# aszepieniec/stark-anatomy

Measured on AMD Instinct MI355X. Metric: ntt_field_elements_per_sec, higher is better.
Workload: dtype u128; 1 GPU; ntt_fwd_inv_2^20_1gpu; log2n=20, parallelism=single, passes_per_transform=2

## Files before the change

stark-anatomy_amd/csrc/field_asm.cuh:

```cuda
#pragma once

#if defined(__HIP_DEVICE_COMPILE__)
namespace sc {

typedef uint64_t smask_t;

#ifndef SC_HAZ_NOP
#define SC_HAZ_NOP "s_nop 1\n\t"
#endif

__device__ __forceinline__ uint64_t a_mad(uint32_t a, uint32_t b, uint64_t c) {
    uint64_t d; smask_t cy;
    asm("v_mad_u64_u32 %0, %1, %2, %3, %4" : "=v"(d), "=s"(cy) : "v"(a), "v"(b), "v"(c));
    return d;
}
__device__ __forceinline__ uint64_t a_madc(uint32_t a, uint32_t b, uint64_t c, smask_t& cy) {
    uint64_t d;
    asm("v_mad_u64_u32 %0, %1, %2, %3, %4" : "=v"(d), "=s"(cy) : "v"(a), "v"(b), "v"(c));
    return d;
}
__device__ __forceinline__ uint32_t a_add_co(uint32_t x, uint32_t y, smask_t& co) {
    uint32_t s;
    asm("v_add_co_u32_e64 %0, %1, %2, %3" : "=v"(s), "=s"(co) : "v"(x), "v"(y));
    return s;
}
__device__ __forceinline__ uint32_t a_addc(uint32_t x, uint32_t y, smask_t ci, smask_t& co) {
    uint32_t s;
    asm(SC_HAZ_NOP "v_addc_co_u32_e64 %0, %1, %2, %3, %4" : "=v"(s), "=s"(co) : "v"(x), "v"(y), "s"(ci));
    return s;
}
__device__ __forceinline__ uint32_t a_addc_last(uint32_t x, uint32_t y, smask_t ci) {
    uint32_t s; smask_t co;
    asm(SC_HAZ_NOP "v_addc_co_u32_e64 %0, %1, %2, %3, %4" : "=v"(s), "=s"(co) : "v"(x), "v"(y), "s"(ci));
    return s;
}
__device__ __forceinline__ uint32_t a_inc(uint32_t x, smask_t ci) {
    uint32_t s; smask_t co;
    asm(SC_HAZ_NOP "v_addc_co_u32_e64 %0, %1, 0, %2, %3" : "=v"(s), "=s"(co) : "v"(x), "s"(ci));
    return s;
}
__device__ __forceinline__ uint32_t a_sub_co(uint32_t x, uint32_t y, smask_t& bo) {
    uint32_t s;
    asm("v_sub_co_u32_e64 %0, %1, %2, %3" : "=v"(s), "=s"(bo) : "v"(x), "v"(y));
    return s;
}
__device__ __forceinline__ uint32_t a_subb(uint32_t x, uint32_t y, smask_t bi, smask_t& bo) {
    uint32_t s;
    asm(SC_HAZ_NOP "v_subb_co_u32_e64 %0, %1, %2, %3, %4" : "=v"(s), "=s"(bo) : "v"(x), "v"(y), "s"(bi));
    return s;
}
__device__ __forceinline__ uint32_t a_negb(uint32_t y, smask_t bi, smask_t& bo) {
    uint32_t s;
    asm(SC_HAZ_NOP "v_subb_co_u32_e64 %0, %1, 0, %2, %3" : "=v"(s), "=s"(bo) : "v"(y), "s"(bi));
    return s;
}
__device__ __forceinline__ uint32_t a_cnd(uint32_t a, uint32_t b, smask_t sel) {
    uint32_t r;
    asm(SC_HAZ_NOP "v_cndmask_b32_e64 %0, %1, %2, %3" : "=v"(r) : "v"(a), "v"(b), "s"(sel));
    return r;
}

__device__ __forceinline__ void rare_or(smask_t& rare, smask_t c) { asm volatile("s_or_b64 %0, %0, %1" : "+s"(rare) : "s"(c) : "scc"); }
__device__ __forceinline__ bool rare_any_asm(smask_t rare) {
    uint32_t any;
    asm("s_cmp_lg_u64 %1, 0\n\ts_cselect_b32 %0, 1, 0" : "=s"(any) : "s"(rare) : "scc");
    return __builtin_amdgcn_readfirstlane(any) != 0;
}

__device__ __forceinline__ uint32_t lo32(uint64_t x) { return (uint32_t)x; }
__device__ __forceinline__ uint32_t hi32(uint64_t x) { return (uint32_t)(x >> 32); }

static constexpr uint32_t PH3 = 0xCB800000u;

__device__ __forceinline__ Fe a_cond_sub_p(uint32_t r0, uint32_t r1, uint32_t r2, uint32_t r3, smask_t cf) {
    smask_t b;
    uint32_t d0 = a_sub_co(r0, 1u, b);
    uint32_t d1 = a_subb(r1, 0u, b, b);
    uint32_t d2 = a_subb(r2, 0u, b, b);
    uint32_t d3 = a_subb(r3, PH3, b, b);
    smask_t sel = cf | ~b;
    uint32_t o0 = a_cnd(r0, d0, sel), o1 = a_cnd(r1, d1, sel), o2 = a_cnd(r2, d2, sel), o3 = a_cnd(r3, d3, sel);
    return Fe{((uint64_t)o1 << 32) | o0, ((uint64_t)o3 << 32) | o2};
}

__device__ __forceinline__ Fe a_fixup_fast(uint32_t d0, uint32_t d1, uint32_t d2, uint32_t d3, smask_t bw, smask_t& rare) {
    smask_t c;
    const uint32_t d3p = d3 + PH3;
    uint32_t o0 = a_addc(d0, 0u, bw, c);
    uint32_t o3 = a_cnd(d3, d3p, bw);
    rare_or(rare, c);
    return Fe{((uint64_t)d1 << 32) | o0, ((uint64_t)o3 << 32) | d2};
}

#define SC_FIX_CARRY(o1, o2, o3, c)                                                \
    SC_HAZ_NOP "v_addc_co_u32_e64 %[" o1 "], %[t], %[" o1 "], 0, %[" c "]\n\t"      \
    SC_HAZ_NOP "v_addc_co_u32_e64 %[" o2 "], %[t], %[" o2 "], 0, %[t]\n\t"          \
    SC_HAZ_NOP "v_addc_co_u32_e64 %[" o3 "], %[t], %[" o3 "], 0, %[t]\n\t"
#define SC_FIX_BORROW(o0, o1, o2, o3, r3, b, ca)                                   \
    SC_HAZ_NOP "v_subb_co_u32_e64 %[" o1 "], %[t], %[" o1 "], 0, %[" b "]\n\t"      \
    SC_HAZ_NOP "v_subb_co_u32_e64 %[" o2 "], %[t], %[" o2 "], 0, %[t]\n\t"          \
    SC_HAZ_NOP "v_subb_co_u32_e64 %[" o3 "], %[t], %[" o3 "], 0, %[t]\n\t"          \
    "s_andn2_b64 %[t], %[t], %[" ca "]\n\t"                                        \
    SC_HAZ_NOP "v_cndmask_b32_e64 %[" o0 "], %[" o0 "], 0, %[t]\n\t"               \
    "v_cndmask_b32_e64 %[" o1 "], %[" o1 "], 0, %[t]\n\t"                          \
    "v_cndmask_b32_e64 %[" o2 "], %[" o2 "], 0, %[t]\n\t"                          \
    "v_cndmask_b32_e64 %[" o3 "], %[" o3 "], %[" r3 "], %[t]\n\t"

__device__ __forceinline__ Fe a_fixup_fix(uint32_t d0, uint32_t d1, uint32_t d2, uint32_t d3, smask_t bw) {
    smask_t c, t;
    const uint32_t d3p = d3 + PH3;
    uint32_t o0 = a_addc(d0, 0u, bw, c);
    uint32_t o3 = a_cnd(d3, d3p, bw);
    asm("s_cmp_eq_u64 %[c], 0\n\t"
        "s_cbranch_scc1 1f\n\t"
        SC_FIX_CARRY("o1", "o2", "o3", "c")
        "1:"
        : [o1] "+v"(d1), [o2] "+v"(d2), [o3] "+v"(o3), [t] "=&s"(t)
        : [c] "s"(c)
        : "scc");
    return Fe{((uint64_t)d1 << 32) | o0, ((uint64_t)o3 << 32) | d2};
}

template <int MODE>
__device__ __forceinline__ Fe mont_mul_core(Fe a, Fe b, smask_t& rare) {
    const uint32_t a0 = lo32(a.lo), a1 = hi32(a.lo), a2 = lo32(a.hi), a3 = hi32(a.hi);
    const uint32_t b0 = lo32(b.lo), b1 = hi32(b.lo), b2 = lo32(b.hi), b3 = hi32(b.hi);
    smask_t c;
    uint64_t E0 = a_mad(a0, b0, 0);
    uint64_t O0 = a_mad(a0, b1, 0);
    O0 = a_madc(a1, b0, O0, c);
    uint32_t nO0 = a_inc(0u, c);
    uint64_t E1 = a_mad(a0, b2, 0);
    E1 = a_madc(a1, b1, E1, c);
    uint32_t nE1 = a_inc(0u, c);
    E1 = a_madc(a2, b0, E1, c);
    nE1 = a_inc(nE1, c);
    uint64_t O1 = a_mad(a0, b3, (uint64_t)nO0);
    O1 = a_madc(a1, b2, O1, c);
    uint32_t nO1 = a_inc(0u, c);
    O1 = a_madc(a2, b1, O1, c);
    nO1 = a_inc(nO1, c);
    O1 = a_madc(a3, b0, O1, c);
    nO1 = a_inc(nO1, c);
    uint64_t E2 = a_mad(a1, b3, (uint64_t)nE1);
    E2 = a_madc(a2, b2, E2, c);
    uint32_t nE2 = a_inc(0u, c);
    E2 = a_madc(a3, b1, E2, c);
    nE2 = a_inc(nE2, c);
    uint64_t O2 = a_mad(a2, b3, (uint64_t)nO1);
    O2 = a_madc(a3, b2, O2, c);
    uint32_t nO2 = a_inc(0u, c);
    uint64_t E3 = a_mad(a3, b3, (uint64_t)nE2);
    const uint32_t t0 = lo32(E0);
    uint32_t t1 = a_add_co(hi32(E0), lo32(O0), c);
    uint32_t t2 = a_addc(lo32(E1), hi32(O0), c, c);
    uint32_t t3 = a_addc(hi32(E1), lo32(O1), c, c);
    uint32_t t4 = a_addc(lo32(E2), hi32(O1), c, c);
    uint32_t t5 = a_addc(hi32(E2), lo32(O2), c, c);
    uint32_t t6 = a_addc(lo32(E3), hi32(O2), c, c);
    uint32_t t7 = a_addc_last(hi32(E3), nO2, c);
    const uint32_t PHc = PH3;
    uint64_t s0 = a_mad(t0, PHc, 0);
    smask_t bw;
    uint32_t m3 = a_sub_co(t3, lo32(s0), bw);
    uint64_t s1 = a_mad(t1, PHc, (uint64_t)hi32(s0));
    uint64_t s2 = a_mad(t2, PHc, (uint64_t)hi32(s1));
    uint64_t s3 = a_mad(m3, PHc, (uint64_t)hi32(s2));
    uint32_t r0 = a_subb(t4, lo32(s1), bw, bw);
    uint32_t r1 = a_subb(t5, lo32(s2), bw, bw);
    uint32_t r2 = a_subb(t6, lo32(s3), bw, bw);
    uint32_t r3 = a_subb(t7, hi32(s3), bw, bw);
    if constexpr (MODE == 1) return a_fixup_fast(r0, r1, r2, r3, bw, rare);
    if constexpr (MODE == 2) return a_fixup_fix(r0, r1, r2, r3, bw);
    uint32_t ph = a_cnd(0u, PH3, bw);
    uint32_t o0 = a_addc(r0, 0u, bw, c);
    uint32_t o1 = a_addc(r1, 0u, c, c);
    uint32_t o2 = a_addc(r2, 0u, c, c);
    uint32_t o3 = a_addc_last(r3, ph, c);
    return Fe{((uint64_t)o1 << 32) | o0, ((uint64_t)o3 << 32) | o2};
}
__device__ __forceinline__ Fe mont_mul_asm(Fe a, Fe b) {
    smask_t none = 0;
    return mont_mul_core<0>(a, b, none);
}
__device__ __forceinline__ Fe mont_mul_fast_asm(Fe a, Fe b, smask_t& rare) { return mont_mul_core<1>(a, b, rare); }
__device__ __forceinline__ Fe mont_mul_fix_asm(Fe a, Fe b) {
    smask_t none = 0;
    return mont_mul_core<2>(a, b, none);
}

#define SC_V_MAD(d, cy, x, y, c)   asm volatile("v_mad_u64_u32 %0, %1, %2, %3, %4" : "=v"(d), "=s"(cy) : "v"(x), "v"(y), "v"(c))
#define SC_V_INC(d, x, ci, co)     asm volatile("v_addc_co_u32_e64 %0, %1, 0, %2, %3" : "=v"(d), "=s"(co) : "v"(x), "s"(ci))
#define SC_V_ADDCO(d, co, x, y)    asm volatile("v_add_co_u32_e64 %0, %1, %2, %3" : "=v"(d), "=s"(co) : "v"(x), "v"(y))
#define SC_V_ADDC(d, co, x, y, ci) asm volatile("v_addc_co_u32_e64 %0, %1, %2, %3, %4" : "=v"(d), "=s"(co) : "v"(x), "v"(y), "s"(ci))
#define SC_V_SUBCO(d, bo, x, y)    asm volatile("v_sub_co_u32_e64 %0, %1, %2, %3" : "=v"(d), "=s"(bo) : "v"(x), "v"(y))
#define SC_V_SUBB(d, bo, x, y, bi) asm volatile("v_subb_co_u32_e64 %0, %1, %2, %3, %4" : "=v"(d), "=s"(bo) : "v"(x), "v"(y), "s"(bi))
#define SC_V_CND(d, x, y, m)       asm volatile("v_cndmask_b32_e64 %0, %1, %2, %3" : "=v"(d) : "v"(x), "v"(y), "s"(m))
#define SC_V_NOP0()                asm volatile("s_nop 0")

template <int W> __device__ __forceinline__ void v_mad_dump(uint64_t& d, uint32_t x, uint32_t y, uint64_t c) {
    if constexpr (W == 0) asm volatile("v_mad_u64_u32 %0, vcc, %1, %2, %3" : "=v"(d) : "v"(x), "v"(y), "v"(c) : "vcc");
    else asm volatile("v_mad_u64_u32 %0, s[100:101], %1, %2, %3" : "=v"(d) : "v"(x), "v"(y), "v"(c) : "s100", "s101");
}
template <int W> __device__ __forceinline__ void v_inc_dump(uint32_t& d, uint32_t x, smask_t ci) {
    if constexpr (W == 0) asm volatile("v_addc_co_u32_e64 %0, vcc, %1, 0, %2" : "=v"(d) : "v"(x), "s"(ci) : "vcc");
    else asm volatile("v_addc_co_u32_e64 %0, s[100:101], %1, 0, %2" : "=v"(d) : "v"(x), "s"(ci) : "s100", "s101");
}
template <int W> __device__ __forceinline__ void v_addc_dump(uint32_t& d, uint32_t x, uint32_t y, smask_t ci) {
    if constexpr (W == 0) asm volatile("v_addc_co_u32_e64 %0, vcc, %1, %2, %3" : "=v"(d) : "v"(x), "v"(y), "s"(ci) : "vcc");
    else asm volatile("v_addc_co_u32_e64 %0, s[100:101], %1, %2, %3" : "=v"(d) : "v"(x), "v"(y), "s"(ci) : "s100", "s101");
}
#define SC_V_MADD(d, x, y, c)      v_mad_dump<W>(d, x, y, c)
#define SC_V_INCD(d, x, ci)        v_inc_dump<W>(d, x, ci)
#define SC_V_ADDCD(d, x, y, ci)    v_addc_dump<W>(d, x, y, ci)

struct MulState {
    uint32_t a0, a1, a2, a3, b0, b1, b2, b3;
    uint64_t E0, O0, E1, O1, E2, O2, E3, s0, s1, s2, s3;
    uint32_t nO0, nE1, nO1, nE2, nO2, t1, t2, t3, t4, t5, t6, t7, m3, r0, r1, r2, r3, ph, o0, o1, o2, o3;
    smask_t c1, c2, c3, c4, c5, c6, c7, c8, c9, ct, bw, cx;
};

template <int MODE>
__device__ __forceinline__ void mont_mul2_core(Fe xa, Fe wa, Fe xb, Fe wb, Fe& ra, Fe& rb, smask_t& rare) {
    MulState A, B;
    A.a0 = lo32(xa.lo); A.a1 = hi32(xa.lo); A.a2 = lo32(xa.hi); A.a3 = hi32(xa.hi);
    A.b0 = lo32(wa.lo); A.b1 = hi32(wa.lo); A.b2 = lo32(wa.hi); A.b3 = hi32(wa.hi);
    B.a0 = lo32(xb.lo); B.a1 = hi32(xb.lo); B.a2 = lo32(xb.hi); B.a3 = hi32(xb.hi);
    B.b0 = lo32(wb.lo); B.b1 = hi32(wb.lo); B.b2 = lo32(wb.hi); B.b3 = hi32(wb.hi);
    const uint64_t zero64 = 0;
    const uint32_t zero32 = 0, PHc = PH3;
#define SC_BOTH(STEP) { MulState& M = A; [[maybe_unused]] constexpr int W = 0; STEP } { MulState& M = B; [[maybe_unused]] constexpr int W = 1; STEP }
    SC_BOTH(SC_V_MADD(M.E0, M.a0, M.b0, zero64);)
    SC_BOTH(SC_V_MADD(M.O0, M.a0, M.b1, zero64);)
    SC_BOTH(SC_V_MADD(M.E1, M.a0, M.b2, zero64);)
    SC_BOTH(SC_V_MAD(M.O0, M.c1, M.a1, M.b0, M.O0);)
    SC_BOTH(SC_V_MAD(M.E1, M.c2, M.a1, M.b1, M.E1);)
    SC_BOTH(SC_V_MAD(M.E1, M.c3, M.a2, M.b0, M.E1);)
    SC_BOTH(SC_V_INCD(M.nO0, zero32, M.c1);)
    SC_BOTH(SC_V_INCD(M.nE1, zero32, M.c2);)
    SC_BOTH(SC_V_INCD(M.nE1, M.nE1, M.c3);)
    SC_BOTH(SC_V_MADD(M.O1, M.a0, M.b3, (uint64_t)M.nO0 | ((uint64_t)M.nE1 << 32));)
    SC_BOTH(SC_V_MAD(M.O1, M.c4, M.a1, M.b2, M.O1);)
    SC_BOTH(SC_V_MAD(M.O1, M.c5, M.a2, M.b1, M.O1);)
    SC_BOTH(SC_V_INCD(M.nO1, zero32, M.c4);)
    SC_BOTH(SC_V_MAD(M.O1, M.c6, M.a3, M.b0, M.O1);)
    SC_BOTH(SC_V_MADD(M.E2, M.a1, M.b3, zero64);)
    SC_BOTH(SC_V_INCD(M.nO1, M.nO1, M.c5);)
    SC_BOTH(SC_V_MAD(M.E2, M.c7, M.a2, M.b2, M.E2);)
    SC_BOTH(SC_V_INCD(M.nO1, M.nO1, M.c6);)
    SC_BOTH(SC_V_MAD(M.E2, M.c8, M.a3, M.b1, M.E2);)
    SC_BOTH(SC_V_INCD(M.nE2, zero32, M.c7);)
    SC_BOTH(SC_V_MADD(M.E3, M.a3, M.b3, zero64);)
    SC_BOTH(SC_V_INCD(M.nE2, M.nE2, M.c8);)
    SC_BOTH(SC_V_MADD(M.O2, M.a2, M.b3, (uint64_t)M.nO1 | ((uint64_t)M.nE2 << 32));)
    SC_BOTH(SC_V_MAD(M.O2, M.c9, M.a3, M.b2, M.O2);)
    SC_BOTH(SC_V_ADDCO(M.t1, M.ct, hi32(M.E0), lo32(M.O0));)
    SC_BOTH(SC_V_MADD(M.s0, lo32(M.E0), PHc, zero64);)
    SC_BOTH(SC_V_INCD(M.nO2, zero32, M.c9);)
    SC_BOTH(SC_V_ADDC(M.t2, M.ct, lo32(M.E1), hi32(M.O0), M.ct);)
    SC_BOTH(SC_V_MADD(M.s1, M.t1, PHc, (uint64_t)hi32(M.s0));)
    SC_BOTH(SC_V_ADDC(M.t3, M.ct, hi32(M.E1), lo32(M.O1), M.ct);)
    SC_BOTH(SC_V_MADD(M.s2, M.t2, PHc, (uint64_t)hi32(M.s1));)
    SC_BOTH(SC_V_SUBCO(M.m3, M.bw, M.t3, lo32(M.s0));)
    SC_BOTH(SC_V_ADDC(M.t4, M.ct, lo32(M.E2), hi32(M.O1), M.ct);)
    SC_BOTH(SC_V_MADD(M.s3, M.m3, PHc, (uint64_t)hi32(M.s2));)
    SC_BOTH(SC_V_ADDC(M.t5, M.ct, hi32(M.E2), lo32(M.O2), M.ct);)
    SC_BOTH(SC_V_SUBB(M.r0, M.bw, M.t4, lo32(M.s1), M.bw);)
    SC_BOTH(SC_V_ADDC(M.t6, M.ct, lo32(M.E3), hi32(M.O2), M.ct);)
    SC_BOTH(SC_V_SUBB(M.r1, M.bw, M.t5, lo32(M.s2), M.bw);)
    SC_BOTH(SC_V_ADDC(M.t7, M.cx, hi32(M.E3), M.nO2, M.ct);)
    SC_BOTH(SC_V_SUBB(M.r2, M.bw, M.t6, lo32(M.s3), M.bw);)
    SC_V_NOP0();
    SC_BOTH(SC_V_SUBB(M.r3, M.bw, M.t7, hi32(M.s3), M.bw);)
    SC_V_NOP0();
    if constexpr (MODE == 2) {
        A.ph = A.r3 + PHc;
        B.ph = B.r3 + PHc;
        SC_BOTH(SC_V_ADDC(M.o0, M.cx, M.r0, zero32, M.bw);)
        SC_BOTH(SC_V_CND(M.o3, M.r3, M.ph, M.bw);)
        smask_t t;
        asm volatile("s_or_b64 %[t], %[ca], %[cb]\n\t"
                     "s_cbranch_scc0 1f\n\t"
                     SC_FIX_CARRY("a1", "a2", "a3", "ca")
                     SC_FIX_CARRY("b1", "b2", "b3", "cb")
                     "1:"
                     : [a1] "+v"(A.r1), [a2] "+v"(A.r2), [a3] "+v"(A.o3), [b1] "+v"(B.r1), [b2] "+v"(B.r2), [b3] "+v"(B.o3), [t] "=&s"(t)
                     : [ca] "s"(A.cx), [cb] "s"(B.cx)
                     : "scc");
        ra = Fe{((uint64_t)A.r1 << 32) | A.o0, ((uint64_t)A.o3 << 32) | A.r2};
        rb = Fe{((uint64_t)B.r1 << 32) | B.o0, ((uint64_t)B.o3 << 32) | B.r2};
        return;
    }
    if constexpr (MODE == 1) {
        A.ph = A.r3 + PHc;
        B.ph = B.r3 + PHc;
        SC_BOTH(SC_V_ADDC(M.o0, M.cx, M.r0, zero32, M.bw);)
        SC_BOTH(SC_V_CND(M.o3, M.r3, M.ph, M.bw);)
        rare_or(rare, A.cx);
        rare_or(rare, B.cx);
        ra = Fe{((uint64_t)A.r1 << 32) | A.o0, ((uint64_t)A.o3 << 32) | A.r2};
        rb = Fe{((uint64_t)B.r1 << 32) | B.o0, ((uint64_t)B.o3 << 32) | B.r2};
        return;
    }
    SC_BOTH(SC_V_CND(M.ph, zero32, PHc, M.bw);)
    SC_BOTH(SC_V_ADDC(M.o0, M.cx, M.r0, zero32, M.bw);)
    SC_V_NOP0();
    SC_BOTH(SC_V_ADDC(M.o1, M.cx, M.r1, zero32, M.cx);)
    SC_V_NOP0();
    SC_BOTH(SC_V_ADDC(M.o2, M.cx, M.r2, zero32, M.cx);)
    SC_V_NOP0();
    SC_BOTH(SC_V_ADDCD(M.o3, M.r3, M.ph, M.cx);)
#undef SC_BOTH
    ra = Fe{((uint64_t)A.o1 << 32) | A.o0, ((uint64_t)A.o3 << 32) | A.o2};
    rb = Fe{((uint64_t)B.o1 << 32) | B.o0, ((uint64_t)B.o3 << 32) | B.o2};
}
__device__ __forceinline__ void mont_mul2_asm(Fe xa, Fe wa, Fe xb, Fe wb, Fe& ra, Fe& rb) {
    smask_t none = 0;
    mont_mul2_core<0>(xa, wa, xb, wb, ra, rb, none);
}
__device__ __forceinline__ void mont_mul2_fast_asm(Fe xa, Fe wa, Fe xb, Fe wb, Fe& ra, Fe& rb, smask_t& rare) {
    mont_mul2_core<1>(xa, wa, xb, wb, ra, rb, rare);
}
__device__ __forceinline__ void mont_mul2_fix_asm(Fe xa, Fe wa, Fe xb, Fe wb, Fe& ra, Fe& rb) {
    smask_t none = 0;
    mont_mul2_core<2>(xa, wa, xb, wb, ra, rb, none);
}

struct AddSubState {
    uint32_t u0, u1, u2, u3, v0, v1, v2, v3;
    uint32_t r0, r1, r2, r3, t0, t1, t2, t3, d0, d1, d2, d3, ph, e0, e1, e2, e3, s0, s1, s2, s3;
    smask_t ca, cb, bd, ce, sel;
};

__device__ __forceinline__ void fe_addsub2_asm(Fe ua, Fe va, Fe ub, Fe vb, Fe& sa, Fe& da, Fe& sb, Fe& db) {
    AddSubState A, B;
    A.u0 = lo32(ua.lo); A.u1 = hi32(ua.lo); A.u2 = lo32(ua.hi); A.u3 = hi32(ua.hi);
    A.v0 = lo32(va.lo); A.v1 = hi32(va.lo); A.v2 = lo32(va.hi); A.v3 = hi32(va.hi);
    B.u0 = lo32(ub.lo); B.u1 = hi32(ub.lo); B.u2 = lo32(ub.hi); B.u3 = hi32(ub.hi);
    B.v0 = lo32(vb.lo); B.v1 = hi32(vb.lo); B.v2 = lo32(vb.hi); B.v3 = hi32(vb.hi);
    const uint32_t zero32 = 0, one32 = 1, PHc = PH3;
#define SC_BOTH(STEP) { AddSubState& M = A; [[maybe_unused]] constexpr int W = 0; STEP } { AddSubState& M = B; [[maybe_unused]] constexpr int W = 1; STEP }
    SC_BOTH(SC_V_ADDCO(M.r0, M.ca, M.u0, M.v0); SC_V_SUBCO(M.d0, M.bd, M.u0, M.v0);)
    SC_BOTH(SC_V_ADDC(M.r1, M.ca, M.u1, M.v1, M.ca); SC_V_SUBB(M.d1, M.bd, M.u1, M.v1, M.bd);)
    SC_BOTH(SC_V_ADDC(M.r2, M.ca, M.u2, M.v2, M.ca); SC_V_SUBB(M.d2, M.bd, M.u2, M.v2, M.bd);)
    SC_BOTH(SC_V_ADDC(M.r3, M.ca, M.u3, M.v3, M.ca); SC_V_SUBB(M.d3, M.bd, M.u3, M.v3, M.bd);)
    SC_BOTH(SC_V_SUBCO(M.t0, M.cb, M.r0, one32); SC_V_CND(M.ph, zero32, PHc, M.bd);)
    SC_BOTH(SC_V_SUBB(M.t1, M.cb, M.r1, zero32, M.cb); SC_V_ADDC(M.e0, M.ce, M.d0, zero32, M.bd);)
    SC_BOTH(SC_V_SUBB(M.t2, M.cb, M.r2, zero32, M.cb); SC_V_ADDC(M.e1, M.ce, M.d1, zero32, M.ce);)
    SC_BOTH(SC_V_SUBB(M.t3, M.cb, M.r3, PHc, M.cb); SC_V_ADDC(M.e2, M.ce, M.d2, zero32, M.ce);)
    A.sel = A.ca | ~A.cb;
    B.sel = B.ca | ~B.cb;
    SC_BOTH(SC_V_CND(M.s0, M.r0, M.t0, M.sel); SC_V_ADDCD(M.e3, M.d3, M.ph, M.ce);)
    SC_BOTH(SC_V_CND(M.s1, M.r1, M.t1, M.sel);)
    SC_BOTH(SC_V_CND(M.s2, M.r2, M.t2, M.sel);)
    SC_BOTH(SC_V_CND(M.s3, M.r3, M.t3, M.sel);)
#undef SC_BOTH
    sa = Fe{((uint64_t)A.s1 << 32) | A.s0, ((uint64_t)A.s3 << 32) | A.s2};
    da = Fe{((uint64_t)A.e1 << 32) | A.e0, ((uint64_t)A.e3 << 32) | A.e2};
    sb = Fe{((uint64_t)B.s1 << 32) | B.s0, ((uint64_t)B.s3 << 32) | B.s2};
    db = Fe{((uint64_t)B.e1 << 32) | B.e0, ((uint64_t)B.e3 << 32) | B.e2};
}

// ... 155 lines not shown
```

stark-anatomy_amd/csrc/ntt_tile.cuh:

```cuda
#pragma once
#include "field.cuh"

namespace sc {

#ifndef SC_MAX_BLOCKS
#define SC_MAX_BLOCKS 16
#endif

struct PassParams {
    const Fe* in;
    Fe* out;
    int logR, logC;
    int lo_log, mid_log;
    uint64_t in_hi, in_mid, in_lo, in_rs, in_cs;
    int in_split;
    uint64_t in_rs_hi;
    uint64_t out_hi, out_mid, out_lo, out_rs, out_cs;
    int rfast_load;
    const Fe* mt;
    int mt_shift;
    int tw_enable;
    int tw_col_shift;
    uint64_t tw_scale;
    uint64_t tw_col_base, tw_row_k, tw_row_mid;
// ... 260 lines not shown
                        x[i0] = fe_add_fix(u, v);
                        dd[bf] = fe_sub_fix(u, v);
                    } else {
                        x[i0] = fe_add(u, v);
                        dd[bf] = fe_sub(u, v);
                    }
                }
            }
#pragma unroll
            for (int bf = 0; bf < E / 2; ++bf) {
                const int i0 = ((bf >> bit) << (bit + 1)) | (bf & ((1 << bit) - 1));
                const int g = i0 >> S;
                const uint32_t fi_low = (uint32_t)(i0 & (F - 1)) & ((1u << bit) - 1u);
                triv[bf] = last && (bit == 0 || fi_low == 0);
                const uint32_t row_lo = rr[g] & ((1u << sh) - 1u);
                ee[bf] = ((fi_low << sh) | row_lo) << tau;
                if (q == 0 && bf == 0) set_prio(prio, 2);
                if (q == S - 1 && bf == 0) set_prio(prio, 1);
            }
#pragma unroll
            for (int bf = 0; bf < E / 2; bf += 2) {
                const int ia = (((bf >> bit) << (bit + 1)) | (bf & ((1 << bit) - 1))) | (1 << bit);
                if (bf + 1 < E / 2) {
                    const int ib = ((((bf + 1) >> bit) << (bit + 1)) | ((bf + 1) & ((1 << bit) - 1))) | (1 << bit);
                    if (!triv[bf] && !triv[bf + 1]) {
                        mul2<FAST>(dd[bf], tw[(uint64_t)ee[bf] << tw_shift], dd[bf + 1], tw[(uint64_t)ee[bf + 1] << tw_shift], x[ia], x[ib], rare);
                    } else {
                        x[ia] = triv[bf] ? dd[bf] : mul1<FAST>(dd[bf], tw[(uint64_t)ee[bf] << tw_shift], rare);
                        x[ib] = triv[bf + 1] ? dd[bf + 1] : mul1<FAST>(dd[bf + 1], tw[(uint64_t)ee[bf + 1] << tw_shift], rare);
                    }
                } else {
                    x[ia] = triv[bf] ? dd[bf] : mul1<FAST>(dd[bf], tw[(uint64_t)ee[bf] << tw_shift], rare);
                }
            }
            if (q == S - 1) set_prio(prio, 0);
        }
    }
    SC_HD static void set_prio(int enable, int level) {
#if defined(__HIP_DEVICE_COMPILE__)
        if (enable) {
            switch (level) {
                case 3: __builtin_amdgcn_s_setprio(3); break;
                case 2: __builtin_amdgcn_s_setprio(2); break;
                case 1: __builtin_amdgcn_s_setprio(1); break;
                default: __builtin_amdgcn_s_setprio(0); break;
            }
        }
#endif
    }
    SC_HD void scatter_lds(int sh, const Fe* x, Fe* lds) const {
#pragma unroll
        for (int i = 0; i < E; ++i) lds[lds_index(row(i, sh), cc[i >> S], logC)] = x[i];
    }
    SC_HD void load_twd(const PassParams& P, Fe* t) const {
        if constexpr (SPLIT_ADDR) {
            const uint32_t lane = bitrev32(row_of(rr[0], 0, 0), logR) * (uint32_t)(P.tw_row_k * P.twd_stride) + (cc[0] >> P.tw_col_shift);
#pragma unroll
            for (int i = 0; i < E; ++i) {
                const Uc u = group_part(i >> S);
                const uint32_t k = bitrev32(row_of(u.rrem, (uint32_t)(i & (F - 1)), 0), logR);
                const uint64_t colidx = ((((uint64_t)t_lo << logC) | u.c) >> P.tw_col_shift) + P.tw_col_base;
                const uint64_t ju = ((uint64_t)k * P.tw_row_k + (uint64_t)t_mid * P.tw_row_mid) * P.twd_stride + colidx;
#if SC_TWD_NT
                t[i] = load_stream(P.twd + ju + lane);
#else
                t[i] = load_at(P.twd + ju, lane << 4);
#endif
            }
            return;
        }
#pragma unroll
        for (int i = 0; i < E; ++i) {
            const uint32_t k = bitrev32(row(i, 0), logR);
            const uint64_t colidx = ((((uint64_t)t_lo << logC) | cc[i >> S]) >> P.tw_col_shift) + P.tw_col_base;
            t[i] = load_stream(&P.twd[((uint64_t)k * P.tw_row_k + (uint64_t)t_mid * P.tw_row_mid) * P.twd_stride + colidx]);
        }
    }
    SC_HD void scatter_global(const PassParams& P, const Fe* x) const {
        Fe none[E];
        if (P.blk_enable) scatter_global<true>(P, x, none, false);
        else scatter_global<false>(P, x, none, false);
    }
    template <bool ALT, int FAST = ARITH_EXACT>
    SC_HD void scatter_global(const PassParams& P, const Fe* x, const Fe (&twd_prefetched)[E], bool have_prefetched, rare_t* rare = nullptr) const {
        Fe v[E];
#pragma unroll
        for (int i = 0; i < E; ++i) v[i] = x[i];
        if (P.tw_enable) {
            Fe t[E];
            if (P.twd) {
                if (have_prefetched) {
#pragma unroll
                    for (int i = 0; i < E; ++i) t[i] = twd_prefetched[i];
                } else {
                    load_twd(P, t);
                }
            } else {
                Fe a[E], b[E];
#pragma unroll
                for (int i = 0; i < E; ++i) {
                    const uint32_t k = bitrev32(row(i, 0), logR);
                    const uint64_t colidx = ((((uint64_t)t_lo << logC) | cc[i >> S]) >> P.tw_col_shift) + P.tw_col_base;
                    const uint64_t e = colidx * ((uint64_t)k * P.tw_row_k + (uint64_t)t_mid * P.tw_row_mid) * P.tw_scale;
                    a[i] = P.tl[e & 4095u];
                    b[i] = P.th[e >> 12];
                }
// ... 25 lines not shown
#pragma unroll
        for (int i = 0; i < E; ++i) {
            const uint32_t k = bitrev32(row(i, 0), logR), c = cc[i >> S];
            uint64_t j = (uint64_t)t_hi * P.out_hi + (uint64_t)t_mid * P.out_mid + (uint64_t)t_lo * P.out_lo + (uint64_t)k * P.out_rs + (uint64_t)c * P.out_cs;
            if constexpr (ALT) {
                const uint32_t nat = k * P.blk_row_k + t_mid * P.blk_row_mid;
                Fe* dst = P.out_blk[nat >> P.blk_log];
                dst[col_off + j] = v[i];
            } else {
                P.out[col_off + j] = v[i];
            }
        }
    }
};

template <int LOGE, int S, int GLR = -1, int GLC = -1, int FAST = ARITH_EXACT>
SC_HD void ntt_round(const PassParams& P, int sh, bool first, uint32_t tile, uint32_t tid, Fe* lds, const Fe* tw, rare_t* rare = nullptr) {
    constexpr int E = 1 << LOGE;
    Round<LOGE, S, GLR, GLC> R;
    R.setup(P, first, tile, tid);
    Fe x[E];
    if (first) {
        Fe tin[E];
        R.gather_global(P, sh, x, tin);
        R.template finish_global<FAST>(P, sh, x, tin, rare);
    } else {
        R.gather_lds(sh, x, lds);
    }
    R.template butterflies<FAST>(sh, x, tw, 0, P.prune_log, -1, P.prio_balance, rare);
    if (sh == 0) {
        Fe none[E];
        if (P.blk_enable) R.template scatter_global<true, FAST>(P, x, none, false, rare);
        else R.template scatter_global<false, FAST>(P, x, none, false, rare);
    } else {
        R.scatter_lds(sh, x, lds);
    }
}

template <int LOGE, int GLR = -1, int GLC = -1>
SC_HD void ntt_round_dispatch(const PassParams& P, int s, int sh, bool first, uint32_t tile, uint32_t tid, Fe* lds, const Fe* tw) {
    if constexpr (LOGE >= 4) { if (s == 4) { ntt_round<LOGE, 4, GLR, GLC>(P, sh, first, tile, tid, lds, tw); return; } }
    if constexpr (LOGE >= 3) { if (s == 3) { ntt_round<LOGE, 3, GLR, GLC>(P, sh, first, tile, tid, lds, tw); return; } }
    if constexpr (LOGE >= 2) { if (s == 2) { ntt_round<LOGE, 2, GLR, GLC>(P, sh, first, tile, tid, lds, tw); return; } }
    ntt_round<LOGE, 1, GLR, GLC>(P, sh, first, tile, tid, lds, tw);
}

SC_HD void tile_twiddles_to_lds(const PassParams& P, int logR, uint32_t tid, uint32_t nthreads, Fe* tw) {
    const uint32_t count = logR > 0 ? (1u << (logR - 1)) : 0u;
    for (uint32_t i = tid; i < count; i += nthreads) tw[i] = P.mt[(uint64_t)i << P.mt_shift];
}

#define SC_FIXED4_SHAPES(X) X(8, 3) X(7, 4) X(10, 2) X(6, 5) X(9, 3) X(8, 4)
#define SC_FIXED8_SHAPES(X) X(10, 2) X(9, 3) X(8, 4)
template <int LOGE, int GLR, int GLC, int ROUND = 0, bool ALT = false, int FAST = ARITH_EXACT>
struct FixedRounds {
    static constexpr int E = 1 << LOGE;
    static constexpr int NR = (GLR + LOGE - 1) / LOGE;
    static constexpr int S = (ROUND == 0) ? (GLR - LOGE * (NR - 1)) : LOGE;
    static constexpr int DONE = (ROUND == 0) ? 0 : (GLR - LOGE * (NR - 1)) + LOGE * (ROUND - 1);
    static constexpr int SH = GLR - DONE - S;
    static constexpr bool NEXT_WAVE_LOCAL = (ROUND >= 1) && (SH + GLC <= 6);
    static constexpr uint32_t TW_COUNT = 1u << (GLR - 1);

    template <class Sync, class WSync, class Stamp>
    SC_HD static void run(const PassParams& P, uint32_t tile, uint32_t tid, Fe* lds, Fe* tw, Sync sync, WSync wsync, Stamp stamp, bool wave_local) {
        rare_t none = 0;
        run(P, tile, tid, lds, tw, sync, wsync, stamp, wave_local, none);
    }
    template <class Sync, class WSync, class Stamp>
    SC_HD static void run(const PassParams& P, uint32_t tile, uint32_t tid, Fe* lds, Fe* tw, Sync sync, WSync wsync, Stamp stamp, bool wave_local, rare_t& rare) {
        Round<LOGE, S, GLR, GLC> R;
        R.setup(P, ROUND == 0, tile, tid);
        Fe x[E];
        if constexpr (ROUND == 0) {
            Fe tin[E];
            Fe twv = fe_zero();
            if (P.prio_balance == 2) Round<LOGE, S, GLR, GLC>::set_prio(1, 3);
            if (tid < TW_COUNT) twv = P.mt[(uint64_t)tid << P.mt_shift];
            R.gather_global(P, SH, x, tin);
            if (P.prio_balance == 2) Round<LOGE, S, GLR, GLC>::set_prio(1, 0);
            if (tid < TW_COUNT) tw[tid] = twv;
            stamp(1);
            sync();
            stamp(2);
            R.template finish_global<FAST>(P, SH, x, tin, &rare);
        } else {
            R.gather_lds(SH, x, lds);
        }
        Fe tpre[E];
        bool prefetched = false;
        if constexpr (ROUND + 1 == NR && NR > 1) {
            if (P.tw_enable && P.twd) {
                R.load_twd(P, tpre);
                prefetched = true;
            }
        }
        const int prune = (ROUND <= 1) ? P.prune_log : 0;
        R.template butterflies<FAST>(SH, x, tw, 0, prune, ROUND + 1 == NR ? 1 : 0, P.prio_balance == 1 ? 1 : 0, &rare);
        stamp(3 + 2 * ROUND);
        if constexpr (ROUND + 1 < NR) {
            R.scatter_lds(SH, x, lds);
            if (NEXT_WAVE_LOCAL && wave_local) wsync(); else sync();
            stamp(4 + 2 * ROUND);
            FixedRounds<LOGE, GLR, GLC, ROUND + 1, ALT, FAST>::run(P, tile, tid, lds, tw, sync, wsync, stamp, wave_local, rare);
        } else {
            R.template scatter_global<ALT, FAST>(P, x, tpre, prefetched, &rare);
            stamp(4 + 2 * ROUND);
        }
    }
};

inline bool fixed_offsets_fit(const PassParams& P) {
    typedef unsigned __int128 u128;
    const u128 lim = (u128)1 << 32, r1 = (1u << P.logR) - 1u, c1 = (1u << P.logC) - 1u;
    if (!P.in_split && (r1 * P.in_rs + c1 * P.in_cs) * sizeof(Fe) >= lim) return false;
    if (!P.blk_enable && (r1 * P.out_rs + c1 * P.out_cs) * sizeof(Fe) >= lim) return false;
    if (P.tw_enable && P.twd && (r1 * P.tw_row_k * P.twd_stride + (c1 >> P.tw_col_shift)) * sizeof(Fe) >= lim) return false;
    return true;
}

inline bool fast_pass_ok(const PassParams& P) { return !P.coset_enable && P.prune_log == 0; }

struct RoundSched {
    int nrounds;
    int s[16];
    int sh[16];
};
SC_HD RoundSched make_rounds(int logR, int loge) {
    RoundSched rs;
    rs.nrounds = (logR + loge - 1) / loge;
    if (rs.nrounds == 0) rs.nrounds = 1;
    int rem = logR;
    for (int i = 0; i < rs.nrounds; ++i) {
        int s = (i == 0) ? (logR - loge * (rs.nrounds - 1)) : loge;
        if (s < 1) s = (logR == 0) ? 0 : 1;
        rem -= s;
        rs.s[i] = s;
        rs.sh[i] = rem;
    }
    return rs;
}

}
```

Baseline: 47.02 billion field-elements/s.

## Use inline zero/SGPR constants in Montgomery asm and split LDS addressing

Montgomery multiply asm helpers now encode zero addends as inline constants and pass the modulus high word through an SGPR instead of a VGPR. This is meant to free vector registers and avoid materialising zero and constant VGPRs. Separately, LDS gather and scatter in the fixed-round NTT path compute one per-lane base address once and XOR/add compile-time uniform offsets per element, aiming to cut address arithmetic. Both are on by default via macros; the split indexing depends on the per-element offsets matching the original lds_index mapping.

Measured after the change: 47.90 billion field-elements/s (median of 6 runs). +1.9%, better.

```diff
diff --git a/stark-anatomy_amd/csrc/field_asm.cuh b/stark-anatomy_amd/csrc/field_asm.cuh
--- a/stark-anatomy_amd/csrc/field_asm.cuh
+++ b/stark-anatomy_amd/csrc/field_asm.cuh
@@ -71,6 +71,44 @@
 __device__ __forceinline__ uint32_t hi32(uint64_t x) { return (uint32_t)(x >> 32); }
 
 static constexpr uint32_t PH3 = 0xCB800000u;
+
+#ifndef SC_SGPR_CONST
+#define SC_SGPR_CONST 1
+#endif
+#if SC_SGPR_CONST
+#define SC_ZERO_OPND "0"
+#define SC_ZERO_ARG(z)
+#define SC_PH_CONSTRAINT "s"
+#else
+#define SC_ZERO_OPND "%[z]"
+#define SC_ZERO_ARG(value) , [z] "v"(value)
+#define SC_PH_CONSTRAINT "v"
+#endif
+__device__ __forceinline__ uint64_t a_mad0(uint32_t a, uint32_t b) {
+    uint64_t d; smask_t cy;
+    asm("v_mad_u64_u32 %[d], %[cy], %[a], %[b], " SC_ZERO_OPND : [d] "=v"(d), [cy] "=s"(cy) : [a] "v"(a), [b] "v"(b) SC_ZERO_ARG((uint64_t)0));
+    return d;
+}
+__device__ __forceinline__ uint64_t a_mad_ph(uint32_t a, uint64_t c) {
+    uint64_t d; smask_t cy;
+    asm("v_mad_u64_u32 %0, %1, %2, %3, %4" : "=v"(d), "=s"(cy) : "v"(a), SC_PH_CONSTRAINT(PH3), "v"(c));
+    return d;
+}
+__device__ __forceinline__ uint64_t a_mad_ph0(uint32_t a) {
+    uint64_t d; smask_t cy;
+    asm("v_mad_u64_u32 %[d], %[cy], %[a], %[ph], " SC_ZERO_OPND : [d] "=v"(d), [cy] "=s"(cy) : [a] "v"(a), [ph] SC_PH_CONSTRAINT(PH3) SC_ZERO_ARG((uint64_t)0));
+    return d;
+}
+__device__ __forceinline__ uint32_t a_inc0(smask_t ci) {
+    uint32_t s; smask_t co;
+    asm(SC_HAZ_NOP "v_addc_co_u32_e64 %[s], %[co], " SC_ZERO_OPND ", 0, %[ci]" : [s] "=v"(s), [co] "=s"(co) : [ci] "s"(ci) SC_ZERO_ARG(0u));
+    return s;
+}
+__device__ __forceinline__ uint32_t a_addc0(uint32_t x, smask_t ci, smask_t& co) {
+    uint32_t s;
+    asm(SC_HAZ_NOP "v_addc_co_u32_e64 %[s], %[co], %[x], " SC_ZERO_OPND ", %[ci]" : [s] "=v"(s), [co] "=s"(co) : [x] "v"(x), [ci] "s"(ci) SC_ZERO_ARG(0u));
+    return s;
+}
 
 __device__ __forceinline__ Fe a_cond_sub_p(uint32_t r0, uint32_t r1, uint32_t r2, uint32_t r3, smask_t cf) {
     smask_t b;
@@ -86,7 +124,7 @@
 __device__ __forceinline__ Fe a_fixup_fast(uint32_t d0, uint32_t d1, uint32_t d2, uint32_t d3, smask_t bw, smask_t& rare) {
     smask_t c;
     const uint32_t d3p = d3 + PH3;
-    uint32_t o0 = a_addc(d0, 0u, bw, c);
+    uint32_t o0 = a_addc0(d0, bw, c);
     uint32_t o3 = a_cnd(d3, d3p, bw);
     rare_or(rare, c);
     return Fe{((uint64_t)d1 << 32) | o0, ((uint64_t)o3 << 32) | d2};
@@ -109,7 +147,7 @@
 __device__ __forceinline__ Fe a_fixup_fix(uint32_t d0, uint32_t d1, uint32_t d2, uint32_t d3, smask_t bw) {
     smask_t c, t;
     const uint32_t d3p = d3 + PH3;
-    uint32_t o0 = a_addc(d0, 0u, bw, c);
+    uint32_t o0 = a_addc0(d0, bw, c);
     uint32_t o3 = a_cnd(d3, d3p, bw);
     asm("s_cmp_eq_u64 %[c], 0\n\t"
         "s_cbranch_scc1 1f\n\t"
@@ -126,30 +164,30 @@
     const uint32_t a0 = lo32(a.lo), a1 = hi32(a.lo), a2 = lo32(a.hi), a3 = hi32(a.hi);
     const uint32_t b0 = lo32(b.lo), b1 = hi32(b.lo), b2 = lo32(b.hi), b3 = hi32(b.hi);
     smask_t c;
-    uint64_t E0 = a_mad(a0, b0, 0);
-    uint64_t O0 = a_mad(a0, b1, 0);
+    uint64_t E0 = a_mad0(a0, b0);
+    uint64_t O0 = a_mad0(a0, b1);
     O0 = a_madc(a1, b0, O0, c);
-    uint32_t nO0 = a_inc(0u, c);
-    uint64_t E1 = a_mad(a0, b2, 0);
+    uint32_t nO0 = a_inc0(c);
+    uint64_t E1 = a_mad0(a0, b2);
     E1 = a_madc(a1, b1, E1, c);
-    uint32_t nE1 = a_inc(0u, c);
+    uint32_t nE1 = a_inc0(c);
     E1 = a_madc(a2, b0, E1, c);
     nE1 = a_inc(nE1, c);
     uint64_t O1 = a_mad(a0, b3, (uint64_t)nO0);
     O1 = a_madc(a1, b2, O1, c);
-    uint32_t nO1 = a_inc(0u, c);
+    uint32_t nO1 = a_inc0(c);
     O1 = a_madc(a2, b1, O1, c);
     nO1 = a_inc(nO1, c);
     O1 = a_madc(a3, b0, O1, c);
     nO1 = a_inc(nO1, c);
     uint64_t E2 = a_mad(a1, b3, (uint64_t)nE1);
     E2 = a_madc(a2, b2, E2, c);
-    uint32_t nE2 = a_inc(0u, c);
+    uint32_t nE2 = a_inc0(c);
     E2 = a_madc(a3, b1, E2, c);
     nE2 = a_inc(nE2, c);
     uint64_t O2 = a_mad(a2, b3, (uint64_t)nO1);
     O2 = a_madc(a3, b2, O2, c);
-    uint32_t nO2 = a_inc(0u, c);
+    uint32_t nO2 = a_inc0(c);
     uint64_t E3 = a_mad(a3, b3, (uint64_t)nE2);
     const uint32_t t0 = lo32(E0);
     uint32_t t1 = a_add_co(hi32(E0), lo32(O0), c);
@@ -159,13 +197,12 @@
     uint32_t t5 = a_addc(hi32(E2), lo32(O2), c, c);
     uint32_t t6 = a_addc(lo32(E3), hi32(O2), c, c);
     uint32_t t7 = a_addc_last(hi32(E3), nO2, c);
-    const uint32_t PHc = PH3;
-    uint64_t s0 = a_mad(t0, PHc, 0);
+    uint64_t s0 = a_mad_ph0(t0);
     smask_t bw;
     uint32_t m3 = a_sub_co(t3, lo32(s0), bw);
-    uint64_t s1 = a_mad(t1, PHc, (uint64_t)hi32(s0));
-    uint64_t s2 = a_mad(t2, PHc, (uint64_t)hi32(s1));
-    uint64_t s3 = a_mad(m3, PHc, (uint64_t)hi32(s2));
+    uint64_t s1 = a_mad_ph(t1, (uint64_t)hi32(s0));
+    uint64_t s2 = a_mad_ph(t2, (uint64_t)hi32(s1));
+    uint64_t s3 = a_mad_ph(m3, (uint64_t)hi32(s2));
     uint32_t r0 = a_subb(t4, lo32(s1), bw, bw);
     uint32_t r1 = a_subb(t5, lo32(s2), bw, bw);
     uint32_t r2 = a_subb(t6, lo32(s3), bw, bw);
@@ -173,9 +210,9 @@
     if constexpr (MODE == 1) return a_fixup_fast(r0, r1, r2, r3, bw, rare);
     if constexpr (MODE == 2) return a_fixup_fix(r0, r1, r2, r3, bw);
     uint32_t ph = a_cnd(0u, PH3, bw);
-    uint32_t o0 = a_addc(r0, 0u, bw, c);
-    uint32_t o1 = a_addc(r1, 0u, c, c);
-    uint32_t o2 = a_addc(r2, 0u, c, c);
+    uint32_t o0 = a_addc0(r0, bw, c);
+    uint32_t o1 = a_addc0(r1, c, c);
+    uint32_t o2 = a_addc0(r2, c, c);
     uint32_t o3 = a_addc_last(r3, ph, c);
     return Fe{((uint64_t)o1 << 32) | o0, ((uint64_t)o3 << 32) | o2};
 }
@@ -213,13 +250,32 @@
 #define SC_V_MADD(d, x, y, c)      v_mad_dump<W>(d, x, y, c)
 #define SC_V_INCD(d, x, ci)        v_inc_dump<W>(d, x, ci)
 #define SC_V_ADDCD(d, x, y, ci)    v_addc_dump<W>(d, x, y, ci)
-
+template <int W> __device__ __forceinline__ void v_mad0_dump(uint64_t& d, uint32_t x, uint32_t y) {
+    if constexpr (W == 0) asm volatile("v_mad_u64_u32 %[d], vcc, %[x], %[y], " SC_ZERO_OPND : [d] "=v"(d) : [x] "v"(x), [y] "v"(y) SC_ZERO_ARG((uint64_t)0) : "vcc");
+    else asm volatile("v_mad_u64_u32 %[d], s[100:101], %[x], %[y], " SC_ZERO_OPND : [d] "=v"(d) : [x] "v"(x), [y] "v"(y) SC_ZERO_ARG((uint64_t)0) : "s100", "s101");
+}
+template <int W> __device__ __forceinline__ void v_madp_dump(uint64_t& d, uint32_t x, uint64_t c) {
+    if constexpr (W == 0) asm volatile("v_mad_u64_u32 %0, vcc, %1, %2, %3" : "=v"(d) : "v"(x), SC_PH_CONSTRAINT(PH3), "v"(c) : "vcc");
+    else asm volatile("v_mad_u64_u32 %0, s[100:101], %1, %2, %3" : "=v"(d) : "v"(x), SC_PH_CONSTRAINT(PH3), "v"(c) : "s100", "s101");
+}
+template <int W> __device__ __forceinline__ void v_madp0_dump(uint64_t& d, uint32_t x) {
+    if constexpr (W == 0) asm volatile("v_mad_u64_u32 %[d], vcc, %[x], %[ph], " SC_ZERO_OPND : [d] "=v"(d) : [x] "v"(x), [ph] SC_PH_CONSTRAINT(PH3) SC_ZERO_ARG((uint64_t)0) : "vcc");
+    else asm volatile("v_mad_u64_u32 %[d], s[100:101], %[x], %[ph], " SC_ZERO_OPND : [d] "=v"(d) : [x] "v"(x), [ph] SC_PH_CONSTRAINT(PH3) SC_ZERO_ARG((uint64_t)0) : "s100", "s101");
+}
+template <int W> __device__ __forceinline__ void v_inc0_dump(uint32_t& d, smask_t ci) {
+    if constexpr (W == 0) asm volatile("v_addc_co_u32_e64 %[d], vcc, " SC_ZERO_OPND ", 0, %[ci]" : [d] "=v"(d) : [ci] "s"(ci) SC_ZERO_ARG(0u) : "vcc");
+    else asm volatile("v_addc_co_u32_e64 %[d], s[100:101], " SC_ZERO_OPND ", 0, %[ci]" : [d] "=v"(d) : [ci] "s"(ci) SC_ZERO_ARG(0u) : "s100", "s101");
+}
+#define SC_V_MADD0(d, x, y)        v_mad0_dump<W>(d, x, y)
+#define SC_V_MADDP(d, x, c)        v_madp_dump<W>(d, x, c)
+#define SC_V_MADDP0(d, x)          v_madp0_dump<W>(d, x)
+#define SC_V_INCD0(d, ci)          v_inc0_dump<W>(d, ci)
+#define SC_V_ADDC0(d, co, x, ci)   asm volatile("v_addc_co_u32_e64 %[s], %[c], %[a], " SC_ZERO_OPND ", %[i]" : [s] "=v"(d), [c] "=s"(co) : [a] "v"(x), [i] "s"(ci) SC_ZERO_ARG(0u))
 struct MulState {
     uint32_t a0, a1, a2, a3, b0, b1, b2, b3;
     uint64_t E0, O0, E1, O1, E2, O2, E3, s0, s1, s2, s3;
     uint32_t nO0, nE1, nO1, nE2, nO2, t1, t2, t3, t4, t5, t6, t7, m3, r0, r1, r2, r3, ph, o0, o1, o2, o3;
-    smask_t c1, c2, c3, c4, c5, c6, c7, c8, c9, ct, bw, cx;
-};
+    smask_t c1, c2, c3, c4, c5, c6, c7, c8, c9, ct, bw, cx;};
 
 template <int MODE>
 __device__ __forceinline__ void mont_mul2_core(Fe xa, Fe wa, Fe xb, Fe wb, Fe& ra, Fe& rb, smask_t& rare) {
@@ -228,43 +284,42 @@
     A.b0 = lo32(wa.lo); A.b1 = hi32(wa.lo); A.b2 = lo32(wa.hi); A.b3 = hi32(wa.hi);
     B.a0 = lo32(xb.lo); B.a1 = hi32(xb.lo); B.a2 = lo32(xb.hi); B.a3 = hi32(xb.hi);
     B.b0 = lo32(wb.lo); B.b1 = hi32(wb.lo); B.b2 = lo32(wb.hi); B.b3 = hi32(wb.hi);
-    const uint64_t zero64 = 0;
-    const uint32_t zero32 = 0, PHc = PH3;
+    [[maybe_unused]] const uint32_t zero32 = 0, PHc = PH3;
 #define SC_BOTH(STEP) { MulState& M = A; [[maybe_unused]] constexpr int W = 0; STEP } { MulState& M = B; [[maybe_unused]] constexpr int W = 1; STEP }
-    SC_BOTH(SC_V_MADD(M.E0, M.a0, M.b0, zero64);)
-    SC_BOTH(SC_V_MADD(M.O0, M.a0, M.b1, zero64);)
-    SC_BOTH(SC_V_MADD(M.E1, M.a0, M.b2, zero64);)
+    SC_BOTH(SC_V_MADD0(M.E0, M.a0, M.b0);)
+    SC_BOTH(SC_V_MADD0(M.O0, M.a0, M.b1);)
+    SC_BOTH(SC_V_MADD0(M.E1, M.a0, M.b2);)
     SC_BOTH(SC_V_MAD(M.O0, M.c1, M.a1, M.b0, M.O0);)
     SC_BOTH(SC_V_MAD(M.E1, M.c2, M.a1, M.b1, M.E1);)
     SC_BOTH(SC_V_MAD(M.E1, M.c3, M.a2, M.b0, M.E1);)
-    SC_BOTH(SC_V_INCD(M.nO0, zero32, M.c1);)
-    SC_BOTH(SC_V_INCD(M.nE1, zero32, M.c2);)
+    SC_BOTH(SC_V_INCD0(M.nO0, M.c1);)
+    SC_BOTH(SC_V_INCD0(M.nE1, M.c2);)
     SC_BOTH(SC_V_INCD(M.nE1, M.nE1, M.c3);)
     SC_BOTH(SC_V_MADD(M.O1, M.a0, M.b3, (uint64_t)M.nO0 | ((uint64_t)M.nE1 << 32));)
     SC_BOTH(SC_V_MAD(M.O1, M.c4, M.a1, M.b2, M.O1);)
     SC_BOTH(SC_V_MAD(M.O1, M.c5, M.a2, M.b1, M.O1);)
-    SC_BOTH(SC_V_INCD(M.nO1, zero32, M.c4);)
+    SC_BOTH(SC_V_INCD0(M.nO1, M.c4);)
     SC_BOTH(SC_V_MAD(M.O1, M.c6, M.a3, M.b0, M.O1);)
-    SC_BOTH(SC_V_MADD(M.E2, M.a1, M.b3, zero64);)
+    SC_BOTH(SC_V_MADD0(M.E2, M.a1, M.b3);)
     SC_BOTH(SC_V_INCD(M.nO1, M.nO1, M.c5);)
     SC_BOTH(SC_V_MAD(M.E2, M.c7, M.a2, M.b2, M.E2);)
     SC_BOTH(SC_V_INCD(M.nO1, M.nO1, M.c6);)
     SC_BOTH(SC_V_MAD(M.E2, M.c8, M.a3, M.b1, M.E2);)
-    SC_BOTH(SC_V_INCD(M.nE2, zero32, M.c7);)
-    SC_BOTH(SC_V_MADD(M.E3, M.a3, M.b3, zero64);)
+    SC_BOTH(SC_V_INCD0(M.nE2, M.c7);)
+    SC_BOTH(SC_V_MADD0(M.E3, M.a3, M.b3);)
     SC_BOTH(SC_V_INCD(M.nE2, M.nE2, M.c8);)
     SC_BOTH(SC_V_MADD(M.O2, M.a2, M.b3, (uint64_t)M.nO1 | ((uint64_t)M.nE2 << 32));)
     SC_BOTH(SC_V_MAD(M.O2, M.c9, M.a3, M.b2, M.O2);)
     SC_BOTH(SC_V_ADDCO(M.t1, M.ct, hi32(M.E0), lo32(M.O0));)
-    SC_BOTH(SC_V_MADD(M.s0, lo32(M.E0), PHc, zero64);)
-    SC_BOTH(SC_V_INCD(M.nO2, zero32, M.c9);)
+    SC_BOTH(SC_V_MADDP0(M.s0, lo32(M.E0));)
+    SC_BOTH(SC_V_INCD0(M.nO2, M.c9);)
     SC_BOTH(SC_V_ADDC(M.t2, M.ct, lo32(M.E1), hi32(M.O0), M.ct);)
-    SC_BOTH(SC_V_MADD(M.s1, M.t1, PHc, (uint64_t)hi32(M.s0));)
+    SC_BOTH(SC_V_MADDP(M.s1, M.t1, (uint64_t)hi32(M.s0));)
     SC_BOTH(SC_V_ADDC(M.t3, M.ct, hi32(M.E1), lo32(M.O1), M.ct);)
-    SC_BOTH(SC_V_MADD(M.s2, M.t2, PHc, (uint64_t)hi32(M.s1));)
+    SC_BOTH(SC_V_MADDP(M.s2, M.t2, (uint64_t)hi32(M.s1));)
     SC_BOTH(SC_V_SUBCO(M.m3, M.bw, M.t3, lo32(M.s0));)
     SC_BOTH(SC_V_ADDC(M.t4, M.ct, lo32(M.E2), hi32(M.O1), M.ct);)
-    SC_BOTH(SC_V_MADD(M.s3, M.m3, PHc, (uint64_t)hi32(M.s2));)
+    SC_BOTH(SC_V_MADDP(M.s3, M.m3, (uint64_t)hi32(M.s2));)
     SC_BOTH(SC_V_ADDC(M.t5, M.ct, hi32(M.E2), lo32(M.O2), M.ct);)
     SC_BOTH(SC_V_SUBB(M.r0, M.bw, M.t4, lo32(M.s1), M.bw);)
     SC_BOTH(SC_V_ADDC(M.t6, M.ct, lo32(M.E3), hi32(M.O2), M.ct);)
@@ -277,7 +332,7 @@
     if constexpr (MODE == 2) {
         A.ph = A.r3 + PHc;
         B.ph = B.r3 + PHc;
-        SC_BOTH(SC_V_ADDC(M.o0, M.cx, M.r0, zero32, M.bw);)
+        SC_BOTH(SC_V_ADDC0(M.o0, M.cx, M.r0, M.bw);)
         SC_BOTH(SC_V_CND(M.o3, M.r3, M.ph, M.bw);)
         smask_t t;
         asm volatile("s_or_b64 %[t], %[ca], %[cb]\n\t"
@@ -295,7 +350,7 @@
     if constexpr (MODE == 1) {
         A.ph = A.r3 + PHc;
         B.ph = B.r3 + PHc;
-        SC_BOTH(SC_V_ADDC(M.o0, M.cx, M.r0, zero32, M.bw);)
+        SC_BOTH(SC_V_ADDC0(M.o0, M.cx, M.r0, M.bw);)
         SC_BOTH(SC_V_CND(M.o3, M.r3, M.ph, M.bw);)
         rare_or(rare, A.cx);
         rare_or(rare, B.cx);
@@ -304,11 +359,11 @@
         return;
     }
     SC_BOTH(SC_V_CND(M.ph, zero32, PHc, M.bw);)
-    SC_BOTH(SC_V_ADDC(M.o0, M.cx, M.r0, zero32, M.bw);)
+    SC_BOTH(SC_V_ADDC0(M.o0, M.cx, M.r0, M.bw);)
     SC_V_NOP0();
-    SC_BOTH(SC_V_ADDC(M.o1, M.cx, M.r1, zero32, M.cx);)
+    SC_BOTH(SC_V_ADDC0(M.o1, M.cx, M.r1, M.cx);)
     SC_V_NOP0();
-    SC_BOTH(SC_V_ADDC(M.o2, M.cx, M.r2, zero32, M.cx);)
+    SC_BOTH(SC_V_ADDC0(M.o2, M.cx, M.r2, M.cx);)
     SC_V_NOP0();
     SC_BOTH(SC_V_ADDCD(M.o3, M.r3, M.ph, M.cx);)
 #undef SC_BOTH
diff --git a/stark-anatomy_amd/csrc/ntt_tile.cuh b/stark-anatomy_amd/csrc/ntt_tile.cuh
--- a/stark-anatomy_amd/csrc/ntt_tile.cuh
+++ b/stark-anatomy_amd/csrc/ntt_tile.cuh
@@ -336,6 +336,45 @@
 #pragma unroll
         for (int i = 0; i < E; ++i) lds[lds_index(row(i, sh), cc[i >> S], logC)] = x[i];
     }
+    template <bool RFAST> SC_HD static Uc uniform_part(int g) {
+        const uint32_t rem = (uint32_t)g << (GLR + GLC - LOGE);
+        if (RFAST) return Uc{rem & ((1u << (GLR - S)) - 1u), rem >> (GLR - S)};
+        return Uc{rem >> GLC, rem & ((1u << GLC) - 1u)};
+    }
+    template <bool RFAST> SC_HD static uint32_t lds_low(int i, int sh) {
+        const Uc u = uniform_part<RFAST>(i >> S);
+        return (u.c ^ row_of(u.rrem, (uint32_t)(i & (F - 1)), sh)) & ((1u << GLC) - 1u);
+    }
+    template <bool RFAST> SC_HD static uint32_t lds_off(int i, int sh) {
+        return row_of(uniform_part<RFAST>(i >> S).rrem, (uint32_t)(i & (F - 1)), sh) << GLC;
+    }
+    SC_HD uint32_t lds_lane(int sh) const { return lds_index(row_of(rr[0], 0, sh), cc[0], logC); }
+    template <bool RFAST> SC_HD static uint32_t lds_index_split(uint32_t lane, int i, int sh) {
+        return (lane ^ lds_low<RFAST>(i, sh)) + lds_off<RFAST>(i, sh);
+    }
+#if defined(__HIP_DEVICE_COMPILE__)
+    typedef __attribute__((address_space(3))) char lchar;
+    typedef __attribute__((address_space(3))) Fe lfe;
+    template <bool RFAST> SC_HD void gather_lds_split(int sh, Fe* x, const Fe* lds) const {
+        const lchar* base = (const lchar*)lds;
+        const uint32_t lane = vgpr_pin(lds_lane(sh) << 4);
+#pragma unroll
+        for (int i = 0; i < E; ++i) x[i] = *reinterpret_cast<const lfe*>(base + ((lane ^ (lds_low<RFAST>(i, sh) << 4)) + (lds_off<RFAST>(i, sh) << 4)));
+    }
+    template <bool RFAST> SC_HD void scatter_lds_split(int sh, const Fe* x, Fe* lds) const {
+        lchar* base = (lchar*)lds;
+        const uint32_t lane = vgpr_pin(lds_lane(sh) << 4);
+#pragma unroll
+        for (int i = 0; i < E; ++i) *reinterpret_cast<lfe*>(base + ((lane ^ (lds_low<RFAST>(i, sh) << 4)) + (lds_off<RFAST>(i, sh) << 4))) = x[i];
+    }
+#else
+    template <bool RFAST> void gather_lds_split(int sh, Fe* x, const Fe* lds) const {
+        for (int i = 0; i < E; ++i) x[i] = lds[lds_index_split<RFAST>(lds_lane(sh), i, sh)];
+    }
+    template <bool RFAST> void scatter_lds_split(int sh, const Fe* x, Fe* lds) const {
+        for (int i = 0; i < E; ++i) lds[lds_index_split<RFAST>(lds_lane(sh), i, sh)] = x[i];
+    }
+#endif
     SC_HD void load_twd(const PassParams& P, Fe* t) const {
         if constexpr (SPLIT_ADDR) {
             const uint32_t lane = bitrev32(row_of(rr[0], 0, 0), logR) * (uint32_t)(P.tw_row_k * P.twd_stride) + (cc[0] >> P.tw_col_shift);
@@ -467,6 +506,9 @@
 
 #define SC_FIXED4_SHAPES(X) X(8, 3) X(7, 4) X(10, 2) X(6, 5) X(9, 3) X(8, 4)
 #define SC_FIXED8_SHAPES(X) X(10, 2) X(9, 3) X(8, 4)
+#ifndef SC_LDS_SPLIT
+#define SC_LDS_SPLIT 1
+#endif
 template <int LOGE, int GLR, int GLC, int ROUND = 0, bool ALT = false, int FAST = ARITH_EXACT>
 struct FixedRounds {
     static constexpr int E = 1 << LOGE;
@@ -476,6 +518,7 @@
     static constexpr int SH = GLR - DONE - S;
     static constexpr bool NEXT_WAVE_LOCAL = (ROUND >= 1) && (SH + GLC <= 6);
     static constexpr uint32_t TW_COUNT = 1u << (GLR - 1);
+    static constexpr bool LDS_SPLIT = SC_LDS_SPLIT && Round<LOGE, S, GLR, GLC>::SPLIT_ADDR;
 
     template <class Sync, class WSync, class Stamp>
     SC_HD static void run(const PassParams& P, uint32_t tile, uint32_t tid, Fe* lds, Fe* tw, Sync sync, WSync wsync, Stamp stamp, bool wave_local) {
@@ -500,7 +543,8 @@
             stamp(2);
             R.template finish_global<FAST>(P, SH, x, tin, &rare);
         } else {
-            R.gather_lds(SH, x, lds);
+            if constexpr (LDS_SPLIT) R.template gather_lds_split<false>(SH, x, lds);
+            else R.gather_lds(SH, x, lds);
         }
         Fe tpre[E];
         bool prefetched = false;
@@ -514,7 +558,12 @@
         R.template butterflies<FAST>(SH, x, tw, 0, prune, ROUND + 1 == NR ? 1 : 0, P.prio_balance == 1 ? 1 : 0, &rare);
         stamp(3 + 2 * ROUND);
         if constexpr (ROUND + 1 < NR) {
-            R.scatter_lds(SH, x, lds);
+            if constexpr (LDS_SPLIT) {
+                if (ROUND == 0 && R.rfast) R.template scatter_lds_split<true>(SH, x, lds);
+                else R.template scatter_lds_split<false>(SH, x, lds);
+            } else {
+                R.scatter_lds(SH, x, lds);
+            }
             if (NEXT_WAVE_LOCAL && wave_local) wsync(); else sync();
             stamp(4 + 2 * ROUND);
             FixedRounds<LOGE, GLR, GLC, ROUND + 1, ALT, FAST>::run(P, tile, tid, lds, tw, sync, wsync, stamp, wave_local, rare);
```
